# MyNiuuu/MOFA-Video

Hardware: AMD Instinct MI355X
Metric: denoised frames/sec, 25f 576x1024 SVD+MOFA, 25 steps (higher is better)
Workload: dtype f16; 1 GPU; MOFA-Video-Traj, 25-frame 576x1024, 25 denoise steps + temporal VAE decode (chunk 8), single trajectory hint, SVD-XT UNet + MOFA-Adapter, CFG 1->3, seeded random weights in the reference checkpoint layout; num_frames=25, height=576, width=1024, num_inference_steps=25, decode_chunk_size=8, parallelism=1 GPU, graph_steps=False, output_finite=True

## Files before the change

mofa_video_amd/csrc/igemm320.hip:

```cpp
#include "igemm_common.h"
#include "igemm_pipe.h"

namespace {

constexpr int WN3 = 2, MI3 = 2;
constexpr int TBM3 = 256;
constexpr int RBH = 64;
constexpr int XPL = TBM3 * RBH;
constexpr int NJ3 = 5;
constexpr int TBN3 = WN3 * NJ3 * 32;
constexpr int PLANE = (TBM3 + TBN3) * RBH;
constexpr int SLOT = 2 * PLANE;
constexpr int BIAS0 = 2 * SLOT;
constexpr int LDS_BYTES3 = BIAS0 + 8 * 2 * 768;
constexpr int LOOKAHEAD3 = 4 + NJ3;

struct ScratchRows { __device__ __forceinline__ int operator()(int r) const { return (r >> 3) * 8192 + (r & 7) * 128; } };

struct Cursor3 {
    int local;
    int ikc, ksw, ky, kx;
    int gx0, gx1;
    unsigned xo0, xo1;
    int phase;
    int kend;
    unsigned wo0;
};

template <int EPI, bool SPLIT = false, bool STATS = false>
__global__ __launch_bounds__(512, 2) void igemm320_f16_kernel(const mofa_igemm_args a, const int tilesN, const int ntiles,
                                                              const Aux aux) {
    constexpr bool R1 = (EPI & EPI_R1) != 0, R2 = (EPI & EPI_R2) != 0, RV = (EPI & EPI_RV) != 0, GEGLU = (EPI & EPI_GEGLU) != 0;
    extern __shared__ __attribute__((aligned(16))) char smem[];
    TileWalk walk;
    walk.init(ntiles);
    const bool has_item = SPLIT && (int)blockIdx.x < aux.nitems;
    if (walk.local >= walk.count && !has_item) return;
    const int tid = threadIdx.x, lane = tid & 63;
    const int wave = __builtin_amdgcn_readfirstlane(tid >> 6);
    const int grp = wave >> 2;
    const int wm = wave / WN3, wn = wave - wm * WN3;
    const int l31 = lane & 31, lh = lane >> 5;

    const int taps = igemm_taps(a);
    const int kpt = a.Cin / 64, nk = taps * kpt;
    const size_t Ktot = (size_t)taps * a.Cin;

    auto swz_bytes = [&](int l, int p) __attribute__((always_inline)) { return (((l & 3) ^ ((l >> 4) & 3)) * 16 + p * RBH); };
    const TapGeo tg(a);
    const unsigned wd1 = 128u * (unsigned)(Ktot * 2), wd2 = (unsigned)(256 + 16 * (wave & 3) - 16 * wave) * (unsigned)(Ktot * 2);
    constexpr unsigned W_DEAD = 0x80000000u;
    const BufRsrc rsx = buf_rsrc(aux.xbase, aux.x_bytes), rsw = buf_rsrc(a.w, aux.w_bytes);
    const LdsDma16 bglds16;
    auto item_decode = [&](int phase, int local, int& tile, int& kb, int& ke) __attribute__((always_inline)) {
        tile = walk.start + (phase == 0 ? local : 0); kb = 0; ke = nk;
        if constexpr (SPLIT) {
            const int q = fdiv((int)blockIdx.x, aux.nsplit_d), ks = (int)blockIdx.x - q * aux.nsplit;
            const int kb1 = fdiv(ks * nk, aux.nsplit_d), ke1 = fdiv((ks + 1) * nk, aux.nsplit_d);
            const bool it = phase == 1;
            tile = it ? aux.tile0 + q : tile;
            kb = it ? kb1 : 0;
            ke = it ? ke1 : nk;
        }
    };
    auto next_pos = [&](int& phase, int& local) __attribute__((always_inline)) {
        if (phase == 0) {
            local += walk.stride;
            if (local >= walk.count) phase = has_item ? 1 : 2;
        } else {
            phase = 2;
        }
    };
    auto cur_setup = [&](Cursor3& c, const int p) __attribute__((always_inline)) {
        const bool live = c.phase < 2;
        int tile, kb, ke;
        item_decode(c.phase, c.local, tile, kb, ke);
        const int tm = fdiv(tile, aux.tiles_n), tn = tile - tm * tilesN;
        const int l = lane_now(lane), r_l = l >> 2;
        const int g0 = pack_geo(a, aux, tm * TBM3 + 16 * wave + r_l), g1 = pack_geo(a, aux, tm * TBM3 + 16 * (wave + 8) + r_l);
        c.gx0 = live ? g0 : -1;
        c.gx1 = live ? g1 : -1;
        const unsigned wo = (unsigned)(tn * TBN3 + 16 * wave + r_l) * (unsigned)(Ktot * 2) + swz_bytes(l, p);
        c.wo0 = live ? wo : W_DEAD;
        c.ikc = 0; c.ksw = 0; c.ky = 0; c.kx = 0;
        c.kend = ke;
        if constexpr (SPLIT) {
            int tap = fdiv(kb, aux.kpt_d);
            c.ikc = kb - tap * kpt;
            c.ksw = kb;
            if (a.mode == MOFA_MODE_CONV3X3) { c.ky = fdiv(tap, aux.ks_d); c.kx = tap - c.ky * tg.ks; } else c.ky = tap;
            c.xo0 = tap_src(a, aux, tg, c.gx0, c.ky, c.kx, swz_bytes(l, p));
            c.xo1 = tap_src(a, aux, tg, c.gx1, c.ky, c.kx, swz_bytes(l, p));
        }
    };
    auto issue = [&](Cursor3& c, const int p, const int slot) __attribute__((always_inline)) {
        if (c.ikc == 0) {
            const int l = lane_now(lane);
            c.xo0 = tap_src(a, aux, tg, c.gx0, c.ky, c.kx, swz_bytes(l, p));
            c.xo1 = tap_src(a, aux, tg, c.gx1, c.ky, c.kx, swz_bytes(l, p));
        }
        char* pl = smem + slot + p * PLANE;
        const int wk = c.ksw * 128;
        bglds16(rsx, c.xo0, c.ikc * 128, pl + wave * 1024);
        bglds16(rsx, c.xo1, c.ikc * 128, pl + (wave + 8) * 1024);
        bglds16(rsw, c.wo0, wk, pl + XPL + wave * 1024);
        bglds16(rsw, c.wo0 + wd1, wk, pl + XPL + (wave + 8) * 1024);
        if (grp == p) bglds16(rsw, c.wo0 + wd2, wk, pl + XPL + (16 + (wave & 3)) * 1024);
    };
    auto advance = [&](Cursor3& c, const int p) __attribute__((always_inline)) {
        tap_advance(c, a, kpt, tg.ks);
        if (c.ksw == c.kend) { next_pos(c.phase, c.local); cur_setup(c, p); }
    };

    int xa, wa;
    {
        const int sl = (lh ^ ((l31 >> 2) & 3)) * 16;
        xa = (wm * MI3 * 32 + l31) * RBH + sl;
        wa = XPL + (wn * NJ3 * 32 + l31) * RBH + sl;
    }

    const BufRsrc rsb = buf_rsrc(a.bias, a.bias ? (unsigned)a.N * 4u : 0u);
    char* bias_lds = smem + BIAS0 + wave * 1536;
    auto bias_prefetch = [&](int phase_, int local_, int slot) __attribute__((always_inline)) {
        if (phase_ != 0) return;
        int tile_, kb_, ke_;
        item_decode(phase_, local_, tile_, kb_, ke_);
        const int tm_ = fdiv(tile_, aux.tiles_n), tn_ = tile_ - tm_ * tilesN;
        const unsigned n0 = (unsigned)(tn_ * TBN3 + wn * NJ3 * 32 + lane_now(lane));
#pragma unroll
        for (int k = 0; k < 3; ++k)
            __builtin_amdgcn_raw_ptr_buffer_load_lds(rsb, (__attribute__((address_space(3))) void*)(bias_lds + slot * 768 + k * 256), 4,
                                                     (n0 + 64u * k) * 4u, 0, 0, 0);
    };

    Cursor3 ca, cb;
    ca.local = cb.local = walk.local;
    ca.phase = cb.phase = walk.local < walk.count ? 0 : 1;
    cur_setup(ca, 0);
    cur_setup(cb, 1);
    bias_prefetch(walk.local < walk.count ? 0 : 1, walk.local, 0);
    issue(ca, 0, 0); advance(ca, 0);
    issue(cb, 1, 0); advance(cb, 1);
    issue(ca, 0, SLOT); advance(ca, 0);
    wait_vmcnt_only<LOOKAHEAD3>();
    __builtin_amdgcn_s_barrier();

    f32x16 acc[MI3][NJ3];
    f16x8 xf[MI3][2], wf[NJ3][2];
    auto phase = [&](auto pc, const int bo, const int bn) __attribute__((always_inline)) {
        constexpr int P = decltype(pc)::v;
#pragma unroll
        for (int k2 = 0; k2 < 2; ++k2) {
            const int xk = k2 ? (xa ^ 32) : xa, wk = k2 ? (wa ^ 32) : wa;
#pragma unroll
            for (int i = 0; i < MI3; ++i) xf[i][k2] = *(const f16x8*)(smem + xk + P * PLANE + i * 32 * RBH);
#pragma unroll
            for (int j = 0; j < NJ3; ++j) wf[j][k2] = *(const f16x8*)(smem + wk + P * PLANE + j * 32 * RBH);
        }
        __builtin_amdgcn_sched_barrier(0);
        if constexpr (P == 0) { issue(cb, 1, bn); advance(cb, 1); }
        else { issue(ca, 0, bo); advance(ca, 0); }
        wait_vmcnt<LOOKAHEAD3>();
        __builtin_amdgcn_sched_barrier(0);
        __builtin_amdgcn_s_barrier();
        __builtin_amdgcn_sched_barrier(0);
        __builtin_amdgcn_s_setprio(1);
#pragma unroll
        for (int k2 = 0; k2 < 2; ++k2)
#pragma unroll
            for (int i = 0; i < MI3; ++i)
#pragma unroll
                for (int j = 0; j < NJ3; ++j)
                    acc[i][j] = __builtin_amdgcn_mfma_f32_32x32x16_f16(wf[j][k2], xf[i][k2], acc[i][j], 0, 0, 0);
        __builtin_amdgcn_s_setprio(0);
        __builtin_amdgcn_sched_barrier(0);
        __builtin_amdgcn_s_barrier();
        __builtin_amdgcn_sched_barrier(0);
    };

    const ScratchRows srow;
    auto epilogue_light = [&](auto ac, auto wnc, f32x16 (&acc)[MI3][NJ3], const int mw, const int nw, char* eb) __attribute__((always_inline)) {
        constexpr int J0 = decltype(wnc)::v ? 1 : 0;
        constexpr int JS = decltype(wnc)::v ? 0 : 4;
        const int lane_e = lane_now(lane);
        const int lane = lane_e, l31 = lane & 31, lh = lane >> 5;
        f16* out = (f16*)a.out;
        float saccv = a.s_acc;
        asm volatile("" : "+v"(saccv));
        char* wr = eb + srow(l31);
#pragma unroll
        for (int i = 0; i < MI3; ++i) {
#pragma unroll
            for (int pr = 0; pr < 2; ++pr) {
                const int j0 = J0 + 2 * pr;
#pragma unroll
                for (int jj = 0; jj < 2; ++jj)
#pragma unroll
                    for (int g = 0; g < 4; ++g) {
                        f16x4 o;
#pragma unroll
                        for (int e = 0; e < 4; ++e) o[e] = (f16)act_apply(ac, saccv * acc[i][j0 + jj][4 * g + e]);
                        const int c8 = 8 * jj + 2 * g + lh;
                        *(f16x4*)h16_off(wr, l31, c8) = o;
                    }
#pragma unroll
                for (int p = 0; p < 4; ++p) {
                    const H16Piece r = h16_row<8>(eb, srow, lane, p);
                    const int mr = mw + 32 * i + r.row, n = nw + 32 * j0 + 8 * r.blk;
                    if (mr < a.M && n + 8 <= a.N) *(f16x8*)(out + (size_t)mr * a.ldo + n) = r.v;
                }
            }
            {
#pragma unroll
                for (int g = 0; g < 4; ++g) {
                    f16x4 o;
#pragma unroll
                    for (int e = 0; e < 4; ++e) o[e] = (f16)act_apply(ac, saccv * acc[i][JS][4 * g + e]);
                    const int c8 = 2 * g + lh;
                    *(f16x4*)h16_off(wr, l31, c8) = o;
                }
#pragma unroll
                for (int p = 0; p < 2; ++p) {
                    const H16Piece r = h16_row<4>(eb, srow, lane, p);
                    const int mr = mw + 32 * i + r.row, n = nw + 32 * JS + 8 * r.blk;
                    if (mr < a.M && n + 8 <= a.N) *(f16x8*)(out + (size_t)mr * a.ldo + n) = r.v;
                }
            }
        }
        wait_lds();
    };
    auto epilogue_res16 = [&](auto wnc, auto unit, f32x16 (&acc)[MI3][NJ3], const int mw, const int nw, char* eb) __attribute__((always_inline)) {
        constexpr int J0 = decltype(wnc)::v ? 1 : 0;
        constexpr int JS = decltype(wnc)::v ? 0 : 4;
        constexpr bool UNIT = decltype(unit)::v != 0;
        constexpr int PPI = 10, NP = MI3 * PPI;
        const int lane_e = lane_now(lane);
        const int lane = lane_e, l31 = lane & 31, lh = lane >> 5;
        f16* out = (f16*)a.out;
        const f16* r1 = (const f16*)a.r1;
        const f16* r2 = (const f16*)a.r2;
        float s1v = a.s1, s2v = a.s2, saccv = a.s_acc;
        asm volatile("" : "+v"(s1v), "+v"(s2v), "+v"(saccv));
        auto piece_pos = [&](int st, int& mr, int& n) __attribute__((always_inline)) {
            const int i = st / PPI, q = st % PPI;
            if (q < 8) {
                mr = mw + 32 * i + 8 * (q & 3) + (lane >> 3);
                n = nw + 32 * (J0 + 2 * (q >> 2)) + 8 * (lane & 7);
            } else {
                mr = mw + 32 * i + 16 * (q - 8) + (lane >> 2);
                n = nw + 32 * JS + 8 * (lane & 3);
            }
        };
        constexpr int D = (R1 && R2) ? 2 : 5;
        f16x8 L1[D], L2[D];
        auto piece_loads = [&](int st, int slot) __attribute__((always_inline)) {
            int mr, n;
            piece_pos(st, mr, n);
            mr = mr < a.M ? mr : a.M - 1;
            n = n + 8 <= a.N ? n : 0;
            if (R1) L1[slot] = *(const f16x8*)(r1 + (size_t)mr * a.ldr1 + n);
            if (R2) L2[slot] = *(const f16x8*)(r2 + (size_t)mr * a.ldr2 + n);
        };
#pragma unroll
        for (int st = 0; st < D; ++st) piece_loads(st, st);
        auto finish = [&](int st, f16x8 o) __attribute__((always_inline)) {
            int mr, n;
            piece_pos(st, mr, n);
            if constexpr (UNIT) {
                o = o + L1[st % D];
            } else {
#pragma unroll
                for (int e = 0; e < 8; ++e) {
                    float x = (float)o[e];
                    if (R1) x += s1v * (float)L1[st % D][e];
                    if (R2) x += s2v * (float)L2[st % D][e];
                    o[e] = (f16)x;
                }
            }
            if (mr < a.M && n + 8 <= a.N) *(f16x8*)(out + (size_t)mr * a.ldo + n) = o;
            if (st + D < NP) piece_loads(st + D, st % D);
        };
        char* wr = eb + srow(l31);
#pragma unroll
        for (int i = 0; i < MI3; ++i) {
#pragma unroll
            for (int pr = 0; pr < 2; ++pr) {
                const int j0 = J0 + 2 * pr;
#pragma unroll
                for (int jj = 0; jj < 2; ++jj)
#pragma unroll
                    for (int g = 0; g < 4; ++g) {
                        f16x4 o;
#pragma unroll
                        for (int e = 0; e < 4; ++e) o[e] = (f16)(saccv * acc[i][j0 + jj][4 * g + e]);
                        const int c8 = 8 * jj + 2 * g + lh;
                        *(f16x4*)h16_off(wr, l31, c8) = o;
                    }
#pragma unroll
                for (int p = 0; p < 4; ++p) {
                    const H16Piece r = h16_row<8>(eb, srow, lane, p);
                    finish(i * PPI + pr * 4 + p, r.v);
                }
            }
            {
#pragma unroll
                for (int g = 0; g < 4; ++g) {
                    f16x4 o;
#pragma unroll
                    for (int e = 0; e < 4; ++e) o[e] = (f16)(saccv * acc[i][JS][4 * g + e]);
                    const int c8 = 2 * g + lh;
                    *(f16x4*)h16_off(wr, l31, c8) = o;
                }
#pragma unroll
                for (int p = 0; p < 2; ++p) {
                    const H16Piece r = h16_row<4>(eb, srow, lane, p);
                    finish(i * PPI + 8 + p, r.v);
                }
            }
        }
        wait_lds();
    };
    auto epilogue_stats = [&](auto wnc, f32x16 (&acc)[MI3][NJ3], const int mw, const int nw, char* eb) __attribute__((always_inline)) {
        constexpr int J0 = decltype(wnc)::v ? 1 : 0, JS = decltype(wnc)::v ? 0 : 4;
        constexpr int NP = 20;
        const int lane_e = lane_now(lane);
        const int lane = lane_e, l31 = lane & 31, lh = lane >> 5;
        f16* out = (f16*)a.out;
        const f16* r1 = (const f16*)a.r1;
        float saccv = a.s_acc;
        asm volatile("" : "+v"(saccv));
        auto piece_pos = [&](int st, int& mr, int& n) __attribute__((always_inline)) {
            if (st < 16) {
                mr = mw + 32 * ((st >> 2) & 1) + 8 * (st & 3) + (lane >> 3);
                n = nw + 32 * (J0 + 2 * (st >> 3)) + 8 * (lane & 7);
            } else {
                mr = mw + 32 * ((st - 16) >> 1) + 16 * ((st - 16) & 1) + (lane >> 2);
                n = nw + 32 * JS + 8 * (lane & 3);
            }
        };
        constexpr int D = 5;
        f16x8 L1[D];
        auto piece_loads = [&](int st, int slot) __attribute__((always_inline)) {
            int mr, n;
            piece_pos(st, mr, n);
            mr = mr < a.M ? mr : a.M - 1;
            L1[slot] = *(const f16x8*)(r1 + (size_t)mr * a.ldr1 + n);
        };
        if constexpr (R1) {
#pragma unroll
            for (int st = 0; st < D; ++st) piece_loads(st, st);
        }
        float S[4], Q[4];
        const f16x2 one2 = {(f16)1.0f, (f16)1.0f};
        auto finish = [&](int st, f16x8 o) __attribute__((always_inline)) {
            int mr, n;
            piece_pos(st, mr, n);
            if constexpr (R1) o = o + L1[st % D];
            if (mr < a.M) *(f16x8*)(out + (size_t)mr * a.ldo + n) = o;
#pragma unroll
            for (int k = 0; k < 4; ++k) {
                const f16x2 h = {o[2 * k], o[2 * k + 1]};
                S[k] = __builtin_amdgcn_fdot2(h, one2, S[k], false);
                Q[k] = __builtin_amdgcn_fdot2(h, h, Q[k], false);
            }
            asm volatile("" : "+v"(S[0]), "+v"(S[1]), "+v"(S[2]), "+v"(S[3]), "+v"(Q[0]), "+v"(Q[1]), "+v"(Q[2]), "+v"(Q[3]));
            if constexpr (R1) {
                if (st + D < NP) piece_loads(st + D, st % D);
            }
        };
        auto reduce_store = [&](const int from, const int n0, const bool writer) __attribute__((always_inline)) {
#pragma unroll
            for (int o = from; o < 64; o <<= 1) {
                const int src = (lane ^ o) << 2;
#pragma unroll
                for (int k = 0; k < 4; ++k) {
                    S[k] += __builtin_bit_cast(float, __builtin_amdgcn_ds_bpermute(src, __builtin_bit_cast(int, S[k])));
                    Q[k] += __builtin_bit_cast(float, __builtin_amdgcn_ds_bpermute(src, __builtin_bit_cast(int, Q[k])));
                }
            }
            if (writer && mw < a.M) {
                float* sp = a.stats + (size_t)(mw >> 6) * a.N + n0;
                *(f32x4*)sp = (f32x4){S[0], Q[0], S[1], Q[1]};
                *(f32x4*)(sp + 4) = (f32x4){S[2], Q[2], S[3], Q[3]};
            }
        };
        char* wr = eb + srow(l31);
#pragma unroll
        for (int pr = 0; pr < 2; ++pr) {
            const int j0 = J0 + 2 * pr;
#pragma unroll
            for (int k = 0; k < 4; ++k) { S[k] = 0.f; Q[k] = 0.f; }
#pragma unroll
            for (int i = 0; i < MI3; ++i) {
#pragma unroll
                for (int jj = 0; jj < 2; ++jj)
#pragma unroll
                    for (int g = 0; g < 4; ++g) {
                        f16x4 o;
#pragma unroll
                        for (int e = 0; e < 4; ++e) o[e] = (f16)(saccv * acc[i][j0 + jj][4 * g + e]);
                        const int c8 = 8 * jj + 2 * g + lh;
                        *(f16x4*)h16_off(wr, l31, c8) = o;
                    }
#pragma unroll
                for (int p = 0; p < 4; ++p) {
                    const H16Piece r = h16_row<8>(eb, srow, lane, p);
                    finish(pr * 8 + i * 4 + p, r.v);
                }
            }
            reduce_store(8, nw + 32 * j0 + 8 * (lane & 7), lane < 8);
        }
#pragma unroll
        for (int k = 0; k < 4; ++k) { S[k] = 0.f; Q[k] = 0.f; }
#pragma unroll
        for (int i = 0; i < MI3; ++i) {
#pragma unroll
            for (int g = 0; g < 4; ++g) {
                f16x4 o;
#pragma unroll
                for (int e = 0; e < 4; ++e) o[e] = (f16)(saccv * acc[i][JS][4 * g + e]);
                const int c8 = 2 * g + lh;
                *(f16x4*)h16_off(wr, l31, c8) = o;
            }
#pragma unroll
            for (int p = 0; p < 2; ++p) {
                const H16Piece r = h16_row<4>(eb, srow, lane, p);
                finish(16 + i * 2 + p, r.v);
            }
        }
        reduce_store(4, nw + 32 * JS + 8 * (lane & 3), lane < 4);
        wait_lds();
    };
    auto epilogue_geglu = [&](auto s1c, f32x16 (&acc)[MI3][NJ3], const int mw, const int nw, char* eb) __attribute__((always_inline)) {
        constexpr bool SACC1 = decltype(s1c)::v != 0;
        const int lane_e = lane_now(lane);
        const int lane = lane_e, l31 = lane & 31, lh = lane >> 5;
        f16* out = (f16*)a.out;
        float saccv = a.s_acc;
        asm volatile("" : "+v"(saccv));
        const int nout = a.N / 2, no0 = nw / 2;
        char* wr = eb + srow(l31);
        auto product = [&](int i, int j, int g) __attribute__((always_inline)) -> f16x4 {
            f16x4 o;
#pragma unroll
            for (int e = 0; e < 4; ++e) {
                const float val = acc[i][j][4 * g + e], gate = acc[i][j][8 + 4 * g + e];
                if constexpr (SACC1) o[e] = (f16)(val * (gate * gelu_phi_f(gate)));
                else o[e] = (f16)(saccv * val * gelu_erf_f(saccv * gate));
            }
            return o;
        };
#pragma unroll
        for (int i = 0; i < MI3; ++i) {
#pragma unroll
            for (int j = 0; j < 4; ++j)
#pragma unroll
                for (int g = 0; g < 2; ++g) {
                    const int c8 = 4 * j + 2 * g + lh;
                    *(f16x4*)h16_off(wr, l31, c8) = product(i, j, g);
                }
#pragma unroll
            for (int p = 0; p < 4; ++p) {
                const H16Piece r = h16_row<8>(eb, srow, lane, p);
                const int mr = mw + 32 * i + r.row, n = no0 + 8 * r.blk;
                if (mr < a.M && n + 8 <= nout) *(f16x8*)(out + (size_t)mr * a.ldo + n) = r.v;
            }
            {
#pragma unroll
                for (int g = 0; g < 2; ++g) {
                    const int c8 = 2 * g + lh;
                    *(f16x4*)h16_off(wr, l31, c8) = product(i, 4, g);
                }
                const H16Piece r = h16_row<2>(eb, srow, lane, 0);
                const int mr = mw + 32 * i + r.row, n = no0 + 64 + 8 * r.blk;
                if (mr < a.M && n + 8 <= nout) *(f16x8*)(out + (size_t)mr * a.ldo + n) = r.v;
            }
        }
        wait_lds();
    };
    auto epilogue_rows = [&](auto un, f32x16 (&acc)[MI3][NJ3], const int mw, const int nw, char* eb) __attribute__((always_inline)) {
        constexpr bool RVROW = RV && decltype(un)::v == 0;
        constexpr int STEPS = MI3 * NJ3;
        const int lane_e = lane_now(lane);
        const int lane = lane_e, l31 = lane & 31, lh = lane >> 5;
        f16* out = (f16*)a.out;
        const f16* r1 = (const f16*)a.r1;
        const f16* r2 = (const f16*)a.r2;
        float s1v = a.s1, s2v = a.s2, saccv = a.s_acc;
        asm volatile("" : "+v"(s1v), "+v"(s2v), "+v"(saccv));
        int rv_div = a.rv_div, rv_mod_in = a.rv_mod_in, rv_mod_out = a.rv_mod_out;
        asm volatile("" : "+s"(rv_div), "+s"(rv_mod_in), "+s"(rv_mod_out));
        const int piece = lane & 3, rrow = lane >> 2;
        constexpr int REGS = (R1 ? 8 : 0) + (R2 ? 8 : 0) + (RVROW ? 16 : 0);
        constexpr int D = RVROW ? 1 : (REGS <= 8 ? 6 : 3);
        struct StepLoads { f16x8 t1[2], t2[2]; f32x4 rv0[2], rv1[2]; };
        StepLoads L[D];
        auto step_loads = [&](int st, StepLoads& l) __attribute__((always_inline)) {
            const int i = st / NJ3, j = st % NJ3;
            const int n = nw + 32 * j + 8 * piece;
            const int nc = n + 8 <= a.N ? n : 0;
#pragma unroll
            for (int p = 0; p < 2; ++p) {
                int m = mw + 32 * i + 16 * p + rrow;
                m = m < a.M ? m : a.M - 1;
                if (R1) l.t1[p] = *(const f16x8*)(r1 + (size_t)m * a.ldr1 + nc);
                if (R2) l.t2[p] = *(const f16x8*)(r2 + (size_t)m * a.ldr2 + nc);
                if (RVROW) {
                    const int idx = ((m / rv_div) * a.rv_mul + (m % rv_mod_in)) % rv_mod_out;
                    const float* q = a.rowvec + (size_t)idx * a.N + nc;
                    l.rv0[p] = *(const f32x4*)q;
                    l.rv1[p] = *(const f32x4*)(q + 4);
                }
            }
        };
#pragma unroll
        for (int st = 0; st < D; ++st) step_loads(st, L[st]);
        char* wr = eb + srow(l31);
        const int wsw = ((l31 >> 1) & 3) | ((l31 & 1) << 2);
#pragma unroll
        for (int st = 0; st < STEPS; ++st) {
            const int i = st / NJ3, j = st % NJ3;
            StepLoads& l = L[st % D];
#pragma unroll
            for (int g = 0; g < 4; ++g) {
                f32x4 v;
#pragma unroll
                for (int e = 0; e < 4; ++e) v[e] = acc[i][j][4 * g + e];
                *(f32x4*)(wr + (((2 * g + lh) ^ wsw) << 4)) = v;
            }
            const int n = nw + 32 * j + 8 * piece;
#pragma unroll
            for (int p = 0; p < 2; ++p) {
                const int row = 16 * p + rrow;
                const int rsw = ((row >> 1) & 3) | ((row & 1) << 2);
                const f32x4 v0 = *(const f32x4*)(eb + srow(row) + (((2 * piece) ^ rsw) << 4));
                const f32x4 v1 = *(const f32x4*)(eb + srow(row) + (((2 * piece + 1) ^ rsw) << 4));
                f16x8 o;
#pragma unroll
                for (int e = 0; e < 4; ++e) {
                    float x0 = v0[e], x1 = v1[e];
                    if (RVROW) { x0 += l.rv0[p][e]; x1 += l.rv1[p][e]; }
                    x0 *= saccv; x1 *= saccv;
                    if (R1 || R2) { x0 = (float)(f16)x0; x1 = (float)(f16)x1; }
                    if (R1) { x0 += s1v * (float)l.t1[p][e]; x1 += s1v * (float)l.t1[p][4 + e]; }
                    if (R2) { x0 += s2v * (float)l.t2[p][e]; x1 += s2v * (float)l.t2[p][4 + e]; }
                    o[e] = (f16)x0; o[4 + e] = (f16)x1;
                }
                const int m = mw + 32 * i + row;
                if (m < a.M && n + 8 <= a.N) *(f16x8*)(out + (size_t)m * a.ldo + n) = o;
            }
            if (st + D < STEPS) step_loads(st + D, L[st % D]);
        }
        wait_lds();
    };

    auto epilogue_dump = [&](f32x16 (&acc)[MI3][NJ3], float* wst, char* eb) __attribute__((always_inline)) {
        const int lane_e = lane_now(lane);
        const int lane = lane_e, l31 = lane & 31, lh = lane >> 5;
        const int piece = lane & 3, rrow = lane >> 2;
        char* wr = eb + srow(l31);
        const int wsw = ((l31 >> 1) & 3) | ((l31 & 1) << 2);
#pragma unroll
        for (int st = 0; st < MI3 * NJ3; ++st) {
            const int i = st / NJ3, j = st % NJ3;
#pragma unroll
            for (int g = 0; g < 4; ++g) {
                f32x4 v;
#pragma unroll
                for (int e = 0; e < 4; ++e) v[e] = acc[i][j][4 * g + e];
                *(f32x4*)(wr + (((2 * g + lh) ^ wsw) << 4)) = v;
            }
#pragma unroll
            for (int p = 0; p < 2; ++p) {
                const int row = 16 * p + rrow;
                const int rsw = ((row >> 1) & 3) | ((row & 1) << 2);
                const f32x4 v0 = *(const f32x4*)(eb + srow(row) + (((2 * piece) ^ rsw) << 4));
                const f32x4 v1 = *(const f32x4*)(eb + srow(row) + (((2 * piece + 1) ^ rsw) << 4));
                float* d = wst + (size_t)(wm * MI3 * 32 + 32 * i + row) * TBN3 + wn * NJ3 * 32 + 32 * j + 8 * piece;
                *(f32x4*)d = v0;
                *(f32x4*)(d + 4) = v1;
            }
        }
        wait_lds();
    };

    int gt = 0;
    int cph = walk.local < walk.count ? 0 : 1, cl = walk.local, bslot = 0;
    for (; cph < 2; next_pos(cph, cl), bslot ^= 1) {
        int tile, kb, ke;
        item_decode(cph, cl, tile, kb, ke);
        {
            int nph = cph, nl = cl;
            next_pos(nph, nl);
            bias_prefetch(nph, nl, bslot ^ 1);
        }
        const int tm = fdiv(tile, aux.tiles_n), tn = tile - tm * tilesN;
        const int mw = tm * TBM3 + wm * MI3 * 32;
        const int nw = tn * TBN3 + wn * NJ3 * 32;
        int idx_u = -1;
        if constexpr (RV) idx_u = rowvec_uniform_idx<32 * MI3>(a, mw);
        if (SPLIT && cph == 1) {
#pragma unroll
            for (int i = 0; i < MI3; ++i)
#pragma unroll
                for (int j = 0; j < NJ3; ++j)
#pragma unroll
                    for (int r = 0; r < 16; ++r) acc[i][j][r] = 0.0f;
        } else {
            const int lane_e = lane_now(lane);
            const int lh_e = lane_e >> 5;
#pragma unroll
            for (int j = 0; j < NJ3; ++j)
#pragma unroll
                for (int g = 0; g < 4; ++g) {
                    f32x4 b = *(const f32x4*)(bias_lds + bslot * 768 + (32 * j + 8 * g + 4 * lh_e) * 4);
                    if (RV && idx_u >= 0) {
                        int n = nw + 32 * j + 8 * g + 4 * lh_e;
                        n = n + 4 <= a.N ? n : 0;
                        b += *(const f32x4*)(a.rowvec + (size_t)idx_u * a.N + n);
                    }
#pragma unroll
                    for (int e = 0; e < 4; ++e) { acc[0][j][4 * g + e] = b[e]; acc[1][j][4 * g + e] = b[e]; }
                }
        }
        if (grp == 1) __builtin_amdgcn_s_barrier();
        for (int kt = kb; kt < ke; ++kt, ++gt) {
            const int bo = (gt & 1) * SLOT, bn = SLOT - bo;
            phase(IC<0>{}, bo, bn);
            phase(IC<1>{}, bo, bn);
            const int d = (gt & 1) ? -SLOT : SLOT;
            xa += d;
            wa += d;
        }
        if (grp == 0) __builtin_amdgcn_s_barrier();

        char* eb = smem + ((gt - 1) & 1) * SLOT + PLANE + wave * 1024;
        if (SPLIT && cph == 1) {
            epilogue_dump(acc, aux.ws + (size_t)blockIdx.x * (TBM3 * TBN3), eb);
        } else if constexpr (STATS) {
            if (wn == 0) epilogue_stats(IC<0>{}, acc, mw, nw, eb);
            else epilogue_stats(IC<1>{}, acc, mw, nw, eb);
        } else if constexpr (GEGLU) {
            if (a.s_acc == 1.0f) epilogue_geglu(IC<1>{}, acc, mw, nw, eb);
            else epilogue_geglu(IC<0>{}, acc, mw, nw, eb);
        } else if constexpr (R1 || R2) {
            if (RV && idx_u < 0) {
                epilogue_rows(IC<0>{}, acc, mw, nw, eb);
            } else {
                const bool unit = R1 && !R2 && a.s1 == 1.0f;
                if (wn == 0) {
                    if (unit) epilogue_res16(IC<0>{}, IC<1>{}, acc, mw, nw, eb);
                    else epilogue_res16(IC<0>{}, IC<0>{}, acc, mw, nw, eb);
                } else {
                    if (unit) epilogue_res16(IC<1>{}, IC<1>{}, acc, mw, nw, eb);
                    else epilogue_res16(IC<1>{}, IC<0>{}, acc, mw, nw, eb);
                }
            }
        } else if (RV && idx_u < 0) {
            epilogue_rows(IC<0>{}, acc, mw, nw, eb);
        } else if (wn == 0) {
            if (RV || a.act == MOFA_ACT_NONE) epilogue_light(IC<MOFA_ACT_NONE>{}, IC<0>{}, acc, mw, nw, eb);
            else if (a.act == MOFA_ACT_SILU) epilogue_light(IC<MOFA_ACT_SILU>{}, IC<0>{}, acc, mw, nw, eb);
            else if (a.act == MOFA_ACT_RELU) epilogue_light(IC<MOFA_ACT_RELU>{}, IC<0>{}, acc, mw, nw, eb);
            else epilogue_light(IC<MOFA_ACT_GELU>{}, IC<0>{}, acc, mw, nw, eb);
        } else {
            if (RV || a.act == MOFA_ACT_NONE) epilogue_light(IC<MOFA_ACT_NONE>{}, IC<1>{}, acc, mw, nw, eb);
            else if (a.act == MOFA_ACT_SILU) epilogue_light(IC<MOFA_ACT_SILU>{}, IC<1>{}, acc, mw, nw, eb);
            else if (a.act == MOFA_ACT_RELU) epilogue_light(IC<MOFA_ACT_RELU>{}, IC<1>{}, acc, mw, nw, eb);
            else epilogue_light(IC<MOFA_ACT_GELU>{}, IC<1>{}, acc, mw, nw, eb);
        }
    }
    wait_vmcnt_only<0>();
}

typedef void (*igemm320_kern_t)(const mofa_igemm_args, const int, const int, const Aux);

__global__ __launch_bounds__(256) void igemm320_fixup_kernel(const mofa_igemm_args a, const float* __restrict__ ws, const int tile0,
                                                             const int nsplit, const int tilesN, const int R) {
    constexpr int PPR = TBN3 / 8, PPT = TBM3 * PPR;
    const long long total = (long long)R * PPT;
    for (long long idx = (long long)blockIdx.x * 256 + threadIdx.x; idx < total; idx += (long long)gridDim.x * 256) {
        const int r = (int)(idx / PPT), rem = (int)(idx - (long long)r * PPT);
        const int rr = rem / PPR, pc = rem - rr * PPR;
        const int tile = tile0 + r, tm = tile / tilesN, tn = tile - tm * tilesN;
        const int m = tm * TBM3 + rr, n = tn * TBN3 + pc * 8;
        if (m >= a.M || n + 8 > a.N) continue;
        float v[8];
#pragma unroll
        for (int e = 0; e < 8; ++e) v[e] = 0.f;
        for (int sl = 0; sl < nsplit; ++sl) {
            const float* q = ws + ((size_t)(r * nsplit + sl) * TBM3 + rr) * TBN3 + pc * 8;
            const f32x4 p0 = *(const f32x4*)q, p1 = *(const f32x4*)(q + 4);
#pragma unroll
            for (int e = 0; e < 4; ++e) { v[e] += p0[e]; v[4 + e] += p1[e]; }
        }
        if (a.bias) {
#pragma unroll
            for (int e = 0; e < 8; ++e) v[e] += a.bias[n + e];
        }
        if (a.rowvec) {
            const int idx_rv = ((m / a.rv_div) * a.rv_mul + (m % a.rv_mod_in)) % a.rv_mod_out;
            const float* q = a.rowvec + (size_t)idx_rv * a.N + n;
#pragma unroll
            for (int e = 0; e < 8; ++e) v[e] += q[e];
        }
#pragma unroll
        for (int e = 0; e < 8; ++e) v[e] *= a.s_acc;
        if (a.r1 || a.r2) {
#pragma unroll
            for (int e = 0; e < 8; ++e) v[e] = (float)(f16)v[e];
        }
        if (a.r1) {
            const f16x8 t = *(const f16x8*)((const f16*)a.r1 + (size_t)m * a.ldr1 + n);
#pragma unroll
            for (int e = 0; e < 8; ++e) v[e] += a.s1 * (float)t[e];
        }
        if (a.r2) {
            const f16x8 t = *(const f16x8*)((const f16*)a.r2 + (size_t)m * a.ldr2 + n);
#pragma unroll
            for (int e = 0; e < 8; ++e) v[e] += a.s2 * (float)t[e];
        }
        f16x8 o;
#pragma unroll
        for (int e = 0; e < 8; ++e) {
            float x = v[e];
            if (a.act == MOFA_ACT_SILU) x = silu_f(x);
            else if (a.act == MOFA_ACT_RELU) x = fmaxf(x, 0.0f);
            else if (a.act == MOFA_ACT_GELU) x = gelu_erf_f(x);
            o[e] = (f16)x;
        }
        *(f16x8*)((f16*)a.out + (size_t)m * a.ldo + n) = o;
    }
}

__global__ __launch_bounds__(192) void igemm320_tile_stats_kernel(const f16* __restrict__ out, const int ldo, float* __restrict__ stats,
                                                                  const int M, const int N, const int tile0, const int tilesN) {
    const int tile = tile0 + (int)(blockIdx.x >> 2), tm = tile / tilesN, tn = tile - tm * tilesN;
    const int m0 = tm * TBM3 + 64 * (int)(blockIdx.x & 3), n = tn * TBN3 + 2 * (int)threadIdx.x;
    if (m0 >= M || (int)threadIdx.x >= TBN3 / 2 || n + 2 > N) return;
    const f16x2 one2 = {(f16)1.0f, (f16)1.0f};
    float sm = 0.f, q = 0.f;
    const f16* p = out + (size_t)m0 * ldo + n;
#pragma unroll 8
    for (int r = 0; r < 64; ++r) {
        const f16x2 h = *(const f16x2*)(p + (size_t)r * ldo);
        sm = __builtin_amdgcn_fdot2(h, one2, sm, false);
        q = __builtin_amdgcn_fdot2(h, h, q, false);
    }
    float* sp = stats + (size_t)(m0 >> 6) * N + n;
    sp[0] = sm;
    sp[1] = q;
}

}

static const igemm320_kern_t k_igemm320[9] = {igemm320_f16_kernel<0>, igemm320_f16_kernel<1>, igemm320_f16_kernel<2>,
                                               igemm320_f16_kernel<3>, igemm320_f16_kernel<4>, igemm320_f16_kernel<5>,
                                               igemm320_f16_kernel<6>, nullptr, igemm320_f16_kernel<8>};
static const igemm320_kern_t k_igemm320_split[7] = {
    igemm320_f16_kernel<0, true>, igemm320_f16_kernel<1, true>, igemm320_f16_kernel<2, true>, igemm320_f16_kernel<3, true>,
    igemm320_f16_kernel<4, true>, igemm320_f16_kernel<5, true>, igemm320_f16_kernel<6, true>};

static const igemm320_kern_t k_igemm320_stats[7] = {igemm320_f16_kernel<0, false, true>, igemm320_f16_kernel<1, false, true>, nullptr,
                                                     nullptr, igemm320_f16_kernel<4, false, true>, igemm320_f16_kernel<5, false, true>, nullptr};
static const igemm320_kern_t k_igemm320_split_stats[7] = {igemm320_f16_kernel<0, true, true>, igemm320_f16_kernel<1, true, true>, nullptr,
                                                           nullptr, igemm320_f16_kernel<4, true, true>, igemm320_f16_kernel<5, true, true>, nullptr};

int igemm320_init() {
    return mofa_lds_optin(k_igemm320, LDS_BYTES3) == MOFA_OK && mofa_lds_optin(k_igemm320_split, LDS_BYTES3) == MOFA_OK &&
                   mofa_lds_optin(k_igemm320_stats, LDS_BYTES3) == MOFA_OK && mofa_lds_optin(k_igemm320_split_stats, LDS_BYTES3) == MOFA_OK
               ? MOFA_OK
               : MOFA_ELAUNCH;
}

static bool igemm320_eligible(const mofa_igemm_args* a, int kind, int taps) {
    if (kind == 7 || !igemm_pipe_eligible(a, kind, (long long)taps * a->Cin)) return false;
    return (long long)(a->N + TBN3) * taps * a->Cin * 2 < 0x7ff00000LL;
}

bool igemm320_stats_ok(const mofa_igemm_args* a) {
    if (!a || !a->x || !a->w || !a->out || a->M <= 0 || a->N <= 0 || a->Cin <= 0 || a->Cin % 64 != 0) return false;
    if (a->act != MOFA_ACT_NONE || a->r2 || (a->r1 && a->s1 != 1.0f)) return false;
    if (a->M % 64 != 0 || a->N % TBN3 != 0) return false;
    if (a->rowvec && (a->rv_mod_in != 1 || a->rv_div <= 0 || a->rv_div % 64 != 0)) return false;
    if (a->tile != 0 && a->tile != MOFA_TILE_256X320) return false;
    return igemm320_eligible(a, (a->r1 ? 1 : 0) | (a->rowvec ? 4 : 0), igemm_taps(*a));
}

int igemm320_split(long long T, int nk, int n_cu, long long ws_bytes) {
    const long long R = T % n_cu;
    if (ws_bytes <= 0 || R == 0) return 1;
    if (T > n_cu && R * 10 > (long long)n_cu * 6) return 1;
    long long s = n_cu / R;
    if (s > 8) s = 8;
    if (s > nk / 8) s = nk / 8;
    if (s >= 2 && 2.0 * nk * (1.0 - 1.0 / (double)s) < 50.0) s = 1;
    const long long per = (long long)TBM3 * TBN3 * 4;
    while (s >= 2 && R * s * per > ws_bytes) --s;
    return s >= 2 ? (int)s : 1;
}

int igemm320_launch(const mofa_igemm_args* a, int kind, int n_cu, hipStream_t stream) {
    const int taps = igemm_taps(*a);
    if (!igemm320_eligible(a, kind, taps)) return 1;
    constexpr int tbn = TBN3;
    const int tilesM = cdiv(a->M, TBM3), tilesN = cdiv(a->N, tbn);
    const long long nt = (long long)tilesM * tilesN;
    if (nt > 0x7fffffffLL) return MOFA_EINVAL;
    Aux aux = igemm_pipe_aux(a, taps, tilesN);
    const int nk = taps * (a->Cin / 64);
    const bool ws_ok = a->workspace && (((size_t)a->workspace) & 15) == 0;
    const int S = kind == 8 ? 1 : igemm320_split(nt, nk, n_cu, ws_ok ? a->workspace_bytes : 0);
    if (a->stats && (kind > 6 || !k_igemm320_stats[kind] || (((size_t)a->stats) & 15) || !igemm320_stats_ok(a))) return MOFA_EINVAL;
    if (S == 1) {
        hipLaunchKernelGGL(a->stats ? k_igemm320_stats[kind] : k_igemm320[kind], dim3(igemm_grid(nt, n_cu)), dim3(512), LDS_BYTES3, stream, *a, tilesN,
                           (int)nt, aux);
        MOFA_CHECK_LAUNCH();
        return MOFA_OK;
    }
    const long long full = nt - nt % n_cu;
    const int R = (int)(nt - full), items = R * S;
    aux.nsplit = S;
    aux.nsplit_d = fastdiv_make(S);
    aux.tile0 = (int)full;
    aux.nitems = items;
    aux.ws = (float*)a->workspace;
    int grid = full > 0 ? (n_cu / 8) * 8 : ((items + 7) / 8) * 8;
    if (grid < items) return MOFA_EINVAL;
    hipLaunchKernelGGL(a->stats ? k_igemm320_split_stats[kind] : k_igemm320_split[kind], dim3(grid), dim3(512), LDS_BYTES3, stream, *a,
                       tilesN, (int)full, aux);
    MOFA_CHECK_LAUNCH();
    const long long pieces = (long long)R * TBM3 * (tbn / 8);
    hipLaunchKernelGGL(igemm320_fixup_kernel, dim3((int)((pieces + 255) / 256)), dim3(256), 0, stream, *a,
                       (const float*)a->workspace, (int)full, S, tilesN, R);
    MOFA_CHECK_LAUNCH();
    if (a->stats) {
        hipLaunchKernelGGL(igemm320_tile_stats_kernel, dim3(R * 4), dim3(192), 0, stream, (const f16*)a->out, a->ldo, a->stats, a->M,
                           a->N, (int)full, tilesN);
        MOFA_CHECK_LAUNCH();
    }
    return MOFA_OK;
}
```

Before: 4.198 frames/s.

## Switch igemm320 inner loop from 32x32x16 to 16x16x32 MFMA with lane remap

Replaces the 32x32x16 f16 MFMA in the 320-wide implicit GEMM kernel with four 16x16x32 MFMAs per 32x32 sub-tile. To support this it changes the LDS read addressing and swizzle, the bias initialization layout, and adds a permlane16_swap pass after the K loop so the existing 32x32-layout epilogues still work. The aim is to use the smaller MFMA shape, which may offer better throughput or latency on MI355X and fewer LDS reads per step. The cost is the extra accumulator shuffle and register-tuple splitting, which could add register pressure and moves.

Measured after the change: 4.293 frames/s (median of 6 runs). 1.02x the previous value.

```diff
diff --git a/mofa_video_amd/csrc/igemm320.hip b/mofa_video_amd/csrc/igemm320.hip
--- a/mofa_video_amd/csrc/igemm320.hip
+++ b/mofa_video_amd/csrc/igemm320.hip
@@ -16,6 +16,8 @@
 constexpr int LOOKAHEAD3 = 4 + NJ3;
 
 struct ScratchRows { __device__ __forceinline__ int operator()(int r) const { return (r >> 3) * 8192 + (r & 7) * 128; } };
+
+__device__ __forceinline__ int slot_swz(int q) { return q ^ ((q & 1) << 1); }
 
 struct Cursor3 {
     int local;
@@ -46,7 +48,7 @@
     const int kpt = a.Cin / 64, nk = taps * kpt;
     const size_t Ktot = (size_t)taps * a.Cin;
 
-    auto swz_bytes = [&](int l, int p) __attribute__((always_inline)) { return (((l & 3) ^ ((l >> 4) & 3)) * 16 + p * RBH); };
+    auto swz_bytes = [&](int l, int p) __attribute__((always_inline)) { return (((l & 3) ^ slot_swz((l >> 4) & 3)) * 16 + p * RBH); };
     const TapGeo tg(a);
     const unsigned wd1 = 128u * (unsigned)(Ktot * 2), wd2 = (unsigned)(256 + 16 * (wave & 3) - 16 * wave) * (unsigned)(Ktot * 2);
     constexpr unsigned W_DEAD = 0x80000000u;
@@ -114,9 +116,10 @@
 
     int xa, wa;
     {
-        const int sl = (lh ^ ((l31 >> 2) & 3)) * 16;
-        xa = (wm * MI3 * 32 + l31) * RBH + sl;
-        wa = XPL + (wn * NJ3 * 32 + l31) * RBH + sl;
+        const int r = lane & 15, c = lane >> 4;
+        const int rw = 8 * ((r >> 2) & 1) + 4 * (r >> 3) + (r & 3);
+        xa = (wm * MI3 * 32 + r) * RBH + (c ^ slot_swz((r >> 2) & 3)) * 16;
+        wa = XPL + (wn * NJ3 * 32 + rw) * RBH + (c ^ slot_swz((rw >> 2) & 3)) * 16;
     }
 
     const BufRsrc rsb = buf_rsrc(a.bias, a.bias ? (unsigned)a.N * 4u : 0u);
@@ -146,17 +149,13 @@
     __builtin_amdgcn_s_barrier();
 
     f32x16 acc[MI3][NJ3];
-    f16x8 xf[MI3][2], wf[NJ3][2];
+    f16x8 xf[2 * MI3], wf[2 * NJ3];
     auto phase = [&](auto pc, const int bo, const int bn) __attribute__((always_inline)) {
         constexpr int P = decltype(pc)::v;
 #pragma unroll
-        for (int k2 = 0; k2 < 2; ++k2) {
-            const int xk = k2 ? (xa ^ 32) : xa, wk = k2 ? (wa ^ 32) : wa;
-#pragma unroll
-            for (int i = 0; i < MI3; ++i) xf[i][k2] = *(const f16x8*)(smem + xk + P * PLANE + i * 32 * RBH);
-#pragma unroll
-            for (int j = 0; j < NJ3; ++j) wf[j][k2] = *(const f16x8*)(smem + wk + P * PLANE + j * 32 * RBH);
-        }
+        for (int i = 0; i < 2 * MI3; ++i) xf[i] = *(const f16x8*)(smem + xa + P * PLANE + i * 16 * RBH);
+#pragma unroll
+        for (int j = 0; j < 2 * NJ3; ++j) wf[j] = *(const f16x8*)(smem + wa + P * PLANE + j * 16 * RBH);
         __builtin_amdgcn_sched_barrier(0);
         if constexpr (P == 0) { issue(cb, 1, bn); advance(cb, 1); }
         else { issue(ca, 0, bo); advance(ca, 0); }
@@ -166,16 +165,44 @@
         __builtin_amdgcn_sched_barrier(0);
         __builtin_amdgcn_s_setprio(1);
 #pragma unroll
-        for (int k2 = 0; k2 < 2; ++k2)
-#pragma unroll
-            for (int i = 0; i < MI3; ++i)
-#pragma unroll
-                for (int j = 0; j < NJ3; ++j)
-                    acc[i][j] = __builtin_amdgcn_mfma_f32_32x32x16_f16(wf[j][k2], xf[i][k2], acc[i][j], 0, 0, 0);
+        for (int i = 0; i < MI3; ++i)
+#pragma unroll
+            for (int j = 0; j < NJ3; ++j)
+#pragma unroll
+                for (int q = 0; q < 4; ++q) {
+                    f32x4 c = {acc[i][j][4 * q], acc[i][j][4 * q + 1], acc[i][j][4 * q + 2], acc[i][j][4 * q + 3]};
+                    c = __builtin_amdgcn_mfma_f32_16x16x32_f16(wf[2 * j + (q >> 1)], xf[2 * i + (q & 1)], c, 0, 0, 0);
+#pragma unroll
+                    for (int e = 0; e < 4; ++e) acc[i][j][4 * q + e] = c[e];
+                }
         __builtin_amdgcn_s_setprio(0);
         __builtin_amdgcn_sched_barrier(0);
         __builtin_amdgcn_s_barrier();
         __builtin_amdgcn_sched_barrier(0);
+    };
+
+    auto to_layout32 = [&](f32x16 (&acc)[MI3][NJ3]) __attribute__((always_inline)) {
+#pragma unroll
+        for (int i = 0; i < MI3; ++i)
+#pragma unroll
+            for (int j = 0; j < NJ3; ++j)
+#pragma unroll
+                for (int v = 0; v < 2; ++v)
+#pragma unroll
+                    for (int s = 0; s < 4; ++s) {
+                        const float lo = acc[i][j][8 * v + s], hi = acc[i][j][8 * v + 4 + s];
+                        const auto sw = __builtin_amdgcn_permlane16_swap(__builtin_bit_cast(unsigned, lo), __builtin_bit_cast(unsigned, hi), false, false);
+                        const unsigned slo = sw[0], shi = sw[1];
+                        acc[i][j][8 * v + s] = __builtin_bit_cast(float, slo);
+                        acc[i][j][8 * v + 4 + s] = __builtin_bit_cast(float, shi);
+                    }
+    };
+
+    auto pin_tuples = [&](f32x16 (&acc)[MI3][NJ3]) __attribute__((always_inline)) {
+#pragma unroll
+        for (int i = 0; i < MI3; ++i)
+#pragma unroll
+            for (int j = 0; j < NJ3; ++j) asm volatile("" : "+v"(acc[i][j]));
     };
 
     const ScratchRows srow;
@@ -608,21 +635,25 @@
                     for (int r = 0; r < 16; ++r) acc[i][j][r] = 0.0f;
         } else {
             const int lane_e = lane_now(lane);
-            const int lh_e = lane_e >> 5;
+            const int col_e = 8 * ((lane_e >> 4) & 1) + 4 * (lane_e >> 5);
 #pragma unroll
             for (int j = 0; j < NJ3; ++j)
 #pragma unroll
-                for (int g = 0; g < 4; ++g) {
-                    f32x4 b = *(const f32x4*)(bias_lds + bslot * 768 + (32 * j + 8 * g + 4 * lh_e) * 4);
+                for (int v = 0; v < 2; ++v) {
+                    f32x4 b = *(const f32x4*)(bias_lds + bslot * 768 + (32 * j + 16 * v + col_e) * 4);
                     if (RV && idx_u >= 0) {
-                        int n = nw + 32 * j + 8 * g + 4 * lh_e;
+                        int n = nw + 32 * j + 16 * v + col_e;
                         n = n + 4 <= a.N ? n : 0;
                         b += *(const f32x4*)(a.rowvec + (size_t)idx_u * a.N + n);
                     }
 #pragma unroll
-                    for (int e = 0; e < 4; ++e) { acc[0][j][4 * g + e] = b[e]; acc[1][j][4 * g + e] = b[e]; }
-                }
-        }
+                    for (int e = 0; e < 4; ++e) {
+                        acc[0][j][8 * v + e] = b[e]; acc[0][j][8 * v + 4 + e] = b[e];
+                        acc[1][j][8 * v + e] = b[e]; acc[1][j][8 * v + 4 + e] = b[e];
+                    }
+                }
+        }
+        pin_tuples(acc);
         if (grp == 1) __builtin_amdgcn_s_barrier();
         for (int kt = kb; kt < ke; ++kt, ++gt) {
             const int bo = (gt & 1) * SLOT, bn = SLOT - bo;
@@ -633,6 +664,9 @@
             wa += d;
         }
         if (grp == 0) __builtin_amdgcn_s_barrier();
+        pin_tuples(acc);
+        to_layout32(acc);
+        pin_tuples(acc);
 
         char* eb = smem + ((gt - 1) & 1) * SLOT + PLANE + wave * 1024;
         if (SPLIT && cph == 1) {
```
